# GiannisPikoulis/dsml-thesis

Hardware: AMD Instinct MI355X
Metric: DDIM denoise steps/sec (64×64×4 latent, 256² face) at 1/2/4/8 GPUs (higher is better)
Workload: dtype f32; 1 GPU; face_reenactment emotion-conditioned LDM (AffectNet config), DDIM-200 schedule, 16 samples/GPU, 64x64x4 latent, CFG off, eta 0, random-init weights; batch_per_gpu=16, global_batch=16, ddim_steps=200, hipgraph=True

## Files before the change

### dsml_thesis_amd/csrc/igemm.hip

```cpp
#include "ldmk_common.h"
#include <stdlib.h>
#include <type_traits>

#if defined(LDMK_IG_STAMPS) && (LDMK_IG_STAMPS == 1 || LDMK_IG_STAMPS == 3)
#define IG_T(i) do { const unsigned long long t_ = __builtin_amdgcn_s_memtime(); ig_acc[i] += t_ - ig_last; ig_last = t_; } while (0)
#elif defined(LDMK_IG_STAMPS)
#define IG_T(i) do { (void)ig_acc; (void)ig_last; } while (0)
#else
#define IG_T(i) do { } while (0)
#endif

namespace ldmk {

typedef __bf16 bf16x4 __attribute__((ext_vector_type(4)));
typedef __bf16 bf16x8 __attribute__((ext_vector_type(8)));
__device__ __forceinline__ bf16x4 to_bf16x4(const float4& v) {
  return bf16x4{(__bf16)v.x, (__bf16)v.y, (__bf16)v.z, (__bf16)v.w};
}

typedef _Float16 f16x4 __attribute__((ext_vector_type(4)));
typedef _Float16 f16x8 __attribute__((ext_vector_type(8)));
constexpr float H2_A_SCALE = 64.f;
__device__ __forceinline__ void split2h(const float4& v, f16x4& h, f16x4& l) {
  h = f16x4{(_Float16)v.x, (_Float16)v.y, (_Float16)v.z, (_Float16)v.w};
// ... 1298 lines not shown
               "ldmk_igemm: the fused skip connection needs a 3x3 convolution on a slab-GEMM tile, skip channels in multiples of 8");
  LDMK_REQUIRE(a.N % 4 == 0 && a.ldb % 4 == 0, "ldmk_igemm: N and ldb must be multiples of 4");
  LDMK_REQUIRE(a.rows_per_sample > 0, "ldmk_igemm: rows_per_sample");
  LDMK_REQUIRE((long long)a.M * a.ldc < (1LL << 31) && a.ldc > 0, "ldmk_igemm: output exceeds 2^31 elements per batch item (32-bit epilogue offsets)");
  const long long samples = ((long long)a.M + a.rows_per_sample - 1) / a.rows_per_sample;
  if (a.a_mode == LDMK_A_CONV3X3) {
    LDMK_REQUIRE(a.in_h > 0 && a.in_w > 0 && a.out_h > 0 && a.out_w > 0 && a.stride >= 1, "ldmk_igemm: conv geometry");
    LDMK_REQUIRE(a.rows_per_sample == a.out_h * a.out_w, "ldmk_igemm: rows_per_sample != out_h*out_w");
    LDMK_REQUIRE(a.batch <= 1, "ldmk_igemm: batched conv unsupported");
    LDMK_REQUIRE(samples * a.in_h * a.in_w * (a.c0 > a.c1 ? a.c0 : a.c1) < (1LL << 31),
                 "ldmk_igemm: conv input exceeds 2^31 elements (32-bit gather indices)");
  } else {
    LDMK_REQUIRE((long long)a.M * (a.c0 > a.c1 ? a.c0 : a.c1) < (1LL << 31), "ldmk_igemm: A exceeds 2^31 elements per batch item");
  }
  if (a.a_tf == LDMK_TF_AFFINE || a.a_tf == LDMK_TF_AFFINE_SILU) LDMK_REQUIRE(a.tf_coef, "ldmk_igemm: tf_coef missing");
  if (a.a_tf == LDMK_TF_LAYERNORM) {
    LDMK_REQUIRE(a.row_stats && a.ln_gamma && a.ln_beta && a.a_mode == LDMK_A_ROWS, "ldmk_igemm: layernorm prologue args");
  }
  if (a.a_tf == LDMK_TF_LAYERNORM_FOLDED)
    LDMK_REQUIRE(a.row_stats && a.ln_colsum && a.a_mode == LDMK_A_ROWS && !a.stats_out && a.batch <= 1,
                 "ldmk_igemm: folded layernorm needs row_stats, ln_colsum (ldmk_fold_layernorm), rows mode, no stats_out, no batching");
  LDMK_REQUIRE(a.a_tf >= LDMK_TF_NONE && a.a_tf <= LDMK_TF_LAYERNORM_FOLDED, "ldmk_igemm: a_tf=%d", a.a_tf);
  if (a.epi == LDMK_EPI_GEGLU) LDMK_REQUIRE(a.N % 64 == 0 && !a.residual && !a.batch_vec, "ldmk_igemm: GEGLU needs N%%64==0 and no residual");
  if (a.stats_out)
    LDMK_REQUIRE(a.M % 32 == 0 && a.rows_per_sample % 32 == 0 && a.epi == LDMK_EPI_NONE && a.batch <= 1,
                 "ldmk_igemm: stats_out needs M%%32==0, rows_per_sample%%32==0, no GEGLU, no batching");
  LDMK_REQUIRE(a.tile_cfg >= 0 && a.tile_cfg <= kNumCfg + kNumRCfg + kNumSCfg + kNumWCfg + kNumPCfg, "ldmk_igemm: tile_cfg=%d outside [0,%d]",
               a.tile_cfg, kNumCfg + kNumRCfg + kNumSCfg + kNumWCfg + kNumPCfg);
  LDMK_REQUIRE(a.splitk >= 0 && a.splitk <= 64, "ldmk_igemm: splitk=%d outside [0,64]", a.splitk);
  LDMK_REQUIRE(a.compute == LDMK_COMPUTE_F32 || a.compute == LDMK_COMPUTE_BF16 || a.compute == LDMK_COMPUTE_BF16X3 || a.compute == LDMK_COMPUTE_F16X2,
               "ldmk_igemm: compute=%d", a.compute);
  const bool ps_tile = a.tile_cfg > kNumCfg + kNumRCfg + kNumSCfg + kNumWCfg;
  if (a.compute == LDMK_COMPUTE_BF16X3 && !ps_tile) {
    LDMK_REQUIRE(a.w_split && !a.b_trans && a.w_split_ld >= a.K && a.w_split_ld % 8 == 0,
                 "ldmk_igemm: LDMK_COMPUTE_BF16X3 needs w_split (ldmk_pack_wsplit), b_trans = 0, w_split_ld >= K and a multiple of 8");
    LDMK_REQUIRE(3LL * a.N * a.w_split_ld * 2 < (1LL << 32), "ldmk_igemm: w_split exceeds 4 GB per batch entry");
    LDMK_REQUIRE(igemm_fast_gather_ok(a), "ldmk_igemm: LDMK_COMPUTE_BF16X3 needs the fast gather (no zero-insertion, two-source "
                 "upsampling or operands beyond 4 GB)");
  }
  if (a.compute == LDMK_COMPUTE_F16X2) {
    LDMK_REQUIRE(a.tile_cfg <= kNumCfg || ps_tile, "ldmk_igemm: LDMK_COMPUTE_F16X2 runs on the LDS-tiled shapes (tile_cfg 0..6) and the pre-split "
                 "tiles (23..28, 31..33), not tile_cfg=%d", a.tile_cfg);
    LDMK_REQUIRE(!a.a_split && a.w_scale_exp >= -60 && a.w_scale_exp <= 60, "ldmk_igemm: LDMK_COMPUTE_F16X2: a_split is not taken; w_scale_exp=%d", a.w_scale_exp);
    if (!ps_tile) {
      LDMK_REQUIRE(a.w_split && !a.b_trans && a.w_split_ld >= a.K && a.w_split_ld % 8 == 0 && 2LL * a.N * a.w_split_ld * 2 < (1LL << 32),
                   "ldmk_igemm: LDMK_COMPUTE_F16X2 needs w_split (ldmk_pack_wsplit_h2), b_trans = 0, w_split_ld >= K and a multiple of 8, below 4 GB");
// ... 97 lines not shown
```

### dsml_thesis_amd/csrc/igemm_ps.hip

```cpp
#include "ldmk_common.h"
#include <stdlib.h>

namespace ldmk {

typedef __bf16 pbf16x4 __attribute__((ext_vector_type(4)));
typedef __bf16 pbf16x8 __attribute__((ext_vector_type(8)));
typedef unsigned int pu32x4 __attribute__((ext_vector_type(4)));

#ifdef LDMK_PS_PROBES
constexpr bool PS_PROBES = true;
#else
constexpr bool PS_PROBES = false;
#endif
static int ps_probe_bits() {
  if (!PS_PROBES) return 0;
  const int dbg = ps_probe_bits();
  return dbg;
}

constexpr unsigned PS_OOB = 0x80000000u;

__device__ __forceinline__ pu32x4 ps_rsrc(const void* ptr, unsigned bytes) {
  const unsigned long long a = (unsigned long long)ptr;
  pu32x4 r;
// ... 1114 lines not shown
  *reinterpret_cast<pf16x8*>(d) = pf16x8{a0[0], a0[1], a0[2], a0[3], a1[0], a1[1], a1[2], a1[3]};
  *reinterpret_cast<pf16x8*>(d + 1024) = pf16x8{l0[0], l0[1], l0[2], l0[3], l1[0], l1[1], l1[2], l1[3]};
}

template <int NWM, int NWN, int TM, int TN, bool TR>
static int psc_launch(const ldmk_igemm_args& a, int splitk, float* ws, hipStream_t st) {
  constexpr int BM = 32 * TM * NWM, BN = 32 * TN * NWN;
  constexpr size_t lds = (size_t)3 * (BM / 32 + BN / 32) * 2048;
  static_assert(lds <= 160 * 1024, "LDS ring exceeds 160 KiB");
  static bool attr = false;
  if (!attr) {
    (void)hipFuncSetAttribute(reinterpret_cast<const void*>(igemm_psc_kernel<NWM, NWN, TM, TN, TR>), hipFuncAttributeMaxDynamicSharedMemorySize, (int)lds);
    attr = true;
  }
  const int tiles = ((a.M + BM - 1) / BM) * ((a.N + BN - 1) / BN);
  static const int nfast_env = [] { const char* e = getenv("LDMK_PS_NFAST"); return e ? atoi(e) : 1; }();
  static const int lean_env = [] { const char* e = getenv("LDMK_PS_LEAN"); return e ? atoi(e) : 1; }();
  const int nfast = (nfast_env && (a.N + BN - 1) / BN > 1 && (a.M + BM - 1) / BM >= 8 ? 1 : 0) | (lean_env ? 0 : 2);
  hipLaunchKernelGGL((igemm_psc_kernel<NWM, NWN, TM, TN, TR>), dim3(tiles, splitk, 1), dim3(64 * NWM * NWN), lds, st, a, splitk, ws, nfast);
  if (splitk > 1 && !a.raw_slabs) return launch_splitk_reduce(a, splitk, ws, st);
  return check_launch("ldmk_igemm(ps, conv)");
}

const char* igemm_ps_unsupported(const ldmk_igemm_args& a, int pcfg, int splitk) {
  if (a.compute != LDMK_COMPUTE_BF16X3 && a.compute != LDMK_COMPUTE_F16X2) return "the pre-split tiles run the bf16x3 and the f16x2 arithmetic (compute)";
  const int pl = a.compute == LDMK_COMPUTE_F16X2 ? 2 : 3;
  if (pl == 2 && (pcfg == 6 || pcfg == 7)) return "the warp-specialised pre-split tiles (29 / 30) exist in the bf16x3 arithmetic only";
  if (pl == 2 && a.out_ps && !a.range_flag) return "out_ps in the f16x2 arithmetic needs range_flag";
  if (!a.a_ps || !a.w_ps) return "a_ps / w_ps (operands in the PS layout: ldmk_pack_ps, ldmk_ln_stats_ps, out_ps of a producer GEMM)";
  if (a.a_mode == LDMK_A_CONV3X3) {
    if (pl != 2) return "the conv-mode pre-split tile runs the f16x2 arithmetic only";
    if (pcfg != 0 && pcfg != 1 && pcfg != 3 && pcfg != 4) return "conv mode: tile_cfg 23 / 24 / 26 / 27";
    if (a.c1 || a.a1 || a.upsample || a.a_tf != LDMK_TF_NONE || a.out_ps || a.batch > 1 || a.epi != LDMK_EPI_NONE || a.attn_kv_out)
      return "conv mode: one pre-normalised source (ldmk_gn_apply_ps_h2), no upsampling / prologue / out_ps / batching / GEGLU";
    if (a.c0 % 32) return "conv mode: C_in must be a multiple of 32";
    if ((a.c0 / 32) % splitk) return "conv mode: splitk must divide C_in / 32 (K is split on 32-channel chunk boundaries)";
    const long long smp = ((long long)a.M + a.rows_per_sample - 1) / a.rows_per_sample;
    if (((smp * a.in_h * a.in_w + 31) / 32) * (a.c0 / 16) * 2048 >= (1LL << 31)) return "conv mode: input of 2 GiB or more";
  } else if (a.a_mode != LDMK_A_ROWS) {
    return "rows mode or 3x3 convolution";
  }
  if (a.b_trans || a.upsample || a.skip_a0 || (a.splitk_counters && !(ps_probe_bits() & 8))) return "b_trans / upsample / fused skip / in-launch combine";
  if (a.a_tf != LDMK_TF_NONE && a.a_tf != LDMK_TF_LAYERNORM_FOLDED) return "no staging prologue: a_ps is what gets multiplied";
  if (a.K % 32 || a.N % 32) return "K and N must be multiples of 32";
  const long long kb = a.K / 16;
  if ((a.a_mode == LDMK_A_ROWS && (long long)((a.M + 31) / 32) * kb * pl * 1024 >= (1LL << 31)) || (long long)(a.N / 32) * kb * pl * 1024 >= (1LL << 31))
    return "an operand of 2 GiB or more";
  if (a.epi == LDMK_EPI_GEGLU && (!kPsCfg[pcfg].even_tn || splitk > 1)) return "GEGLU needs a tile of (value, gate) pairs (256x256, 128x256) and no split-K";
  if (splitk > a.K / 32) return "more K slices than 32-deep chunks";
  if (a.out_ps) {
    if (splitk > 1 || a.batch > 1 || a.stats_out) return "out_ps: no split-K, no batching, no GroupNorm records (transposed epilogue)";
    if (a.ldc % 16) return "out_ps: ldc (the PS output's column count) must be a multiple of 16";
  } else if (!a.out && splitk <= 1) {
    return "no output";
  }
  if (a.stats_out && !a.out) return "stats_out needs out";
  if (a.attn_kv_out) {
    if (pl != 2 || (pcfg != 0 && pcfg != 4)) return "attn_kv_out: the F16X2 arithmetic on tile_cfg 23 / 27";
    if (a.stats_out || splitk > 1 || a.batch > 1 || a.epi != LDMK_EPI_NONE || a.out_ps || !a.out || !a.range_flag)
      return "attn_kv_out: the fused QKV projection (no split-K / batching / GEGLU / records / out_ps; out and range_flag required)";
    if (a.attn_heads <= 0 || a.N != 3 * 32 * a.attn_heads) return "attn_kv_out: N must be 3 x 32 x attn_heads ([q | k | v] of d_head 32)";
    if (a.attn_tokens <= 0 || a.attn_tokens % 64 || a.M % a.attn_tokens) return "attn_kv_out: attn_tokens a multiple of 64 that divides M";
  }
  return nullptr;
}

int igemm_ps_dispatch(const ldmk_igemm_args& a, int pcfg, int splitk, float* ws, hipStream_t st) {
  const bool tr = !a.stats_out;
  if (a.a_mode == LDMK_A_CONV3X3) {
    switch (pcfg) {
      case 0: return tr ? psc_launch<8, 1, 1, 5, true>(a, splitk, ws, st) : psc_launch<8, 1, 1, 5, false>(a, splitk, ws, st);
      case 1: return tr ? psc_launch<4, 2, 2, 5, true>(a, splitk, ws, st) : psc_launch<4, 2, 2, 5, false>(a, splitk, ws, st);
      case 3: return tr ? psc_launch<4, 2, 1, 5, true>(a, splitk, ws, st) : psc_launch<4, 2, 1, 5, false>(a, splitk, ws, st);
      default: return tr ? psc_launch<4, 1, 1, 5, true>(a, splitk, ws, st) : psc_launch<4, 1, 1, 5, false>(a, splitk, ws, st);
    }
  }
  if (a.compute == LDMK_COMPUTE_F16X2 && a.attn_kv_out)
    return pcfg == 0 ? ps_launch<8, 1, 1, 5, 3, true, 2, true>(a, splitk, ws, st) : ps_launch<4, 1, 1, 5, 3, true, 2, true>(a, splitk, ws, st);
  if (a.compute == LDMK_COMPUTE_F16X2) {
    switch (pcfg) {
      case 0: return tr ? ps_launch<8, 1, 1, 5, 3, true, 2>(a, splitk, ws, st) : ps_launch<8, 1, 1, 5, 3, false, 2>(a, splitk, ws, st);
      case 1: return tr ? ps_launch<4, 2, 2, 5, 3, true, 2>(a, splitk, ws, st) : ps_launch<4, 2, 2, 5, 3, false, 2>(a, splitk, ws, st);
      case 2: return tr ? ps_launch<4, 2, 2, 4, 3, true, 2>(a, splitk, ws, st) : ps_launch<4, 2, 2, 4, 3, false, 2>(a, splitk, ws, st);
      case 3: return tr ? ps_launch<4, 2, 1, 5, 3, true, 2>(a, splitk, ws, st) : ps_launch<4, 2, 1, 5, 3, false, 2>(a, splitk, ws, st);
      case 4: return tr ? ps_launch<4, 1, 1, 5, 3, true, 2>(a, splitk, ws, st) : ps_launch<4, 1, 1, 5, 3, false, 2>(a, splitk, ws, st);
      case 8: return tr ? ps_launch<4, 1, 2, 5, 3, true, 2>(a, splitk, ws, st) : ps_launch<4, 1, 2, 5, 3, false, 2>(a, splitk, ws, st);
      case 9: return tr ? ps_launch<4, 1, 2, 4, 3, true, 2>(a, splitk, ws, st) : ps_launch<4, 1, 2, 4, 3, false, 2>(a, splitk, ws, st);
      case 10: return tr ? ps_launch<2, 2, 2, 4, 3, true, 2>(a, splitk, ws, st) : ps_launch<2, 2, 2, 4, 3, false, 2>(a, splitk, ws, st);
      default: return tr ? ps_launch<4, 2, 1, 4, 3, true, 2>(a, splitk, ws, st) : ps_launch<4, 2, 1, 4, 3, false, 2>(a, splitk, ws, st);
    }
// ... 106 lines not shown
```

### dsml_thesis_amd/engine.py

```python
import ctypes as C
import math
import os

import torch

from . import lib as L
from . import switches


def plan_key(a, m):
    key = f"{m},{a.N},{a.K},{a.a_mode},{a.a_tf},{a.epi},{max(1, a.batch)}"
    if a.b_trans:
        key += ",bt"
    if a.a_mode == L.A_CONV3X3 and (a.stride != 1 or a.upsample):
        key += f",s{a.stride}u{a.upsample}"
    return key


_SECTIONS = {"f32": "LDMK_PLAN_TABLE", "bf16x3": "LDMK_X3_TABLE", "f16x2": "LDMK_H2_TABLE", "ps_bf16x3": "LDMK_PS_TABLE",
             "ps_f16x2": "LDMK_PS_H2_TABLE"}
_TABLES = {}
_PLAN_FILE = os.path.join(os.path.dirname(os.path.abspath(__file__)), "igemm_plans.json")


# ... 570 lines not shown
        a._algo_flops = 2.0 * (4 * pix) * cout * (9 * c)
        if plan is not None:
            pg.igemm_ps(a, *plan)
        else:
            pg.igemm(a, self.pin, batch_is_samples=False)
        part = None
        out2d = out.view(-1, cout)
        if stats:
            self.drop_stats(out2d)
            part = self.stats_buffer(4 * pix, cout)
        pg.add("ldmk_upconv_scatter", p_(Pm), p_(bias), p_(out), p_(part), n, h, w, cout)
        if stats:
            self.attach_stats(out2d, part)
        pg.release(A, Pm)
        return out

    def _maybe_stats(self, a, out2d, rows_per_sample, stats):
        if stats and a.M % 32 == 0 and rows_per_sample % 32 == 0:
            self.drop_stats(out2d)
            part = self.stats_buffer(a.M, a.N)
            a.stats_out = part.data_ptr()
            self.attach_stats(out2d, part)

    def ps_query(self, M, N, K, tf=L.TF_NONE, epi=L.EPI_NONE, batch=1, per_sample=True):
        if not ps_enabled():
            return None
        m = M
        if self.pin is not None and self.pin[0] != self.pin[1] and per_sample:
            m = max(1, M * self.pin[0] // self.pin[1])
        return ps_plan(f"{N},{K},{L.A_ROWS},{tf},{epi},{max(1, batch)}", m, h2=getattr(self.pg, "h2_flag", None) is not None,
                       far=bool(getattr(self.pg, "far_plans", False)))

    def lin_ps(self, plan, M, K, a_ps, wp, w_ps, bias, rows_per_sample, out=None, out_ps=None, geglu=False, stats=False, **kw):
        pg, ops = self.pg, self.ops
        N = wp.shape[1]
        ncol = N // 2 if geglu else N
        if out is None and out_ps is None:
            out = pg.alloc(M, ncol)
        a = ops.make_igemm_args(M, N, K, None, K, wp, out, ncol, rows_per_sample, bias=bias,
                                epi=L.EPI_GEGLU if geglu else L.EPI_NONE, a_ps=a_ps, w_ps=w_ps, out_ps=out_ps,
                                range_flag=getattr(pg, "h2_flag", None), **kw)
        if out is not None:
            self._maybe_stats(a, out, rows_per_sample, stats)
        pg.igemm_ps(a, *plan)
        return out

    def lin(self, x0, wp, bias, rows_per_sample, x1=None, out=None, geglu=False, stats=False, wf=None, **kw):
        pg, ops = self.pg, self.ops
        M, c0 = x0.shape[0], x0.shape[-1]
        c1 = 0 if x1 is None else x1.shape[-1]
        N = wp.shape[1]
        ncol = N // 2 if geglu else N
# ... 29 lines not shown
```

### dsml_thesis_amd/lib.py

```python
import ctypes as C
import os

from . import switches

_HERE = os.path.dirname(os.path.abspath(__file__))
LIB_PATH = switches.get("LDMK_LIBRARY") or os.path.join(_HERE, "libldmk.so")

A_ROWS, A_CONV3X3 = 0, 1
TF_NONE, TF_AFFINE, TF_AFFINE_SILU, TF_LAYERNORM, TF_LAYERNORM_FOLDED = 0, 1, 2, 3, 4
EPI_NONE, EPI_GEGLU = 0, 1
COMPUTE_F32, COMPUTE_BF16, COMPUTE_BF16X3, COMPUTE_F16X2 = 0, 1, 2, 3
POST_NONE, POST_GROUPNORM, POST_LAYERNORM = 0, 1, 2

_fp = C.c_void_p


class IgemmArgs(C.Structure):
    _fields_ = [
        ("M", C.c_int), ("N", C.c_int), ("K", C.c_int),
        ("a0", _fp), ("a1", _fp), ("c0", C.c_int), ("c1", C.c_int),
        ("a_mode", C.c_int), ("in_h", C.c_int), ("in_w", C.c_int), ("out_h", C.c_int), ("out_w", C.c_int),
        ("stride", C.c_int), ("pad_lo", C.c_int), ("upsample", C.c_int),
        ("a_tf", C.c_int), ("tf_coef", _fp), ("row_stats", _fp), ("ln_gamma", _fp), ("ln_beta", _fp),
        ("rows_per_sample", C.c_int),
        ("w", _fp), ("b_trans", C.c_int), ("ldb", C.c_int),
        ("bias", _fp), ("batch_vec", _fp), ("batch_vec_ld", C.c_int),
        ("residual", _fp), ("epi", C.c_int),
        ("out", _fp), ("ldc", C.c_int), ("batch", C.c_int),
        ("a_bstride", C.c_longlong), ("w_bstride", C.c_longlong), ("out_bstride", C.c_longlong),
        ("alpha", C.c_float), ("tile_cfg", C.c_int), ("splitk", C.c_int),
        ("splitk_ws", _fp), ("splitk_ws_elems", C.c_longlong), ("stats_out", _fp), ("compute", C.c_int), ("splitk_counters", _fp), ("splitk_counters_len", C.c_int),
        ("w_frag", _fp),
        ("ln_colsum", _fp),
        ("raw_slabs", C.c_int),
        ("skip_a0", _fp), ("skip_a1", _fp), ("skip_c0", C.c_int), ("skip_c1", C.c_int),
        ("w_split", _fp), ("w_split_ld", C.c_int), ("w_split_bstride", C.c_longlong),
        ("a_split", _fp), ("a_split_ld", C.c_int),
        ("a_ps", _fp), ("a_ps_bstride", C.c_longlong), ("w_ps", _fp), ("w_ps_bstride", C.c_longlong), ("out_ps", _fp),
        ("w_scale_exp", C.c_int), ("range_flag", _fp),
        ("attn_kv_out", _fp), ("attn_tokens", C.c_int), ("attn_heads", C.c_int),
    ]


class PostArgs(C.Structure):
    _fields_ = [
        ("src", _fp), ("nslab", C.c_int), ("slab_stride", C.c_longlong), ("M", C.c_int), ("N", C.c_int),
        ("rows_per_sample", C.c_int), ("alpha", C.c_float), ("bias", _fp), ("batch_vec", _fp), ("batch_vec_ld", C.c_int),
        ("residual", _fp), ("ldr", C.c_int), ("geglu", C.c_int), ("raw_out", _fp), ("ld_raw", C.c_int), ("norm", C.c_int),
        ("x1", _fp), ("c1", C.c_int), ("groups", C.c_int), ("eps", C.c_float), ("gamma", _fp), ("beta", _fp),
        ("silu", C.c_int), ("norm_out", _fp), ("ld_norm", C.c_int), ("gn_cache_floats", C.c_int),
        ("gn_scratch", _fp), ("gn_scratch_elems", C.c_longlong),
    ]


class WgradArgs(C.Structure):
    _fields_ = [
        ("R", C.c_int), ("Kw", C.c_int), ("N", C.c_int), ("a", _fp), ("c", C.c_int), ("lda", C.c_int),
        ("a_mode", C.c_int), ("in_h", C.c_int), ("in_w", C.c_int), ("out_h", C.c_int), ("out_w", C.c_int),
        ("stride", C.c_int), ("pad_lo", C.c_int), ("upsample", C.c_int),
        ("dy", _fp), ("ldy", C.c_int), ("dw", _fp), ("ldw", C.c_int), ("accumulate", C.c_int), ("alpha", C.c_float),
        ("batch", C.c_int), ("a_bstride", C.c_longlong), ("dy_bstride", C.c_longlong), ("dw_bstride", C.c_longlong),
        ("splitr", C.c_int), ("ws", _fp), ("ws_elems", C.c_longlong), ("dbias", _fp), ("compute", C.c_int),
    ]
# ... 164 lines not shown
```

### dsml_thesis_amd/ops.py

```python
import ctypes as C
import math

import weakref

import torch

from . import lib as L


def _ptr(t):
    return 0 if t is None else (t if isinstance(t, int) else t.data_ptr())


def stream():
    return torch.cuda.current_stream().cuda_stream


def _chk(t, name):
    if t is None:
        return
    if not (t.is_cuda and t.dtype == torch.float32 and t.is_contiguous()):
        raise L.LdmkError(f"{name}: expected a contiguous float32 CUDA tensor, got {t.dtype} {t.device} "
                          f"contiguous={t.is_contiguous()}")

# ... 198 lines not shown
    a.geglu = 1 if geglu else 0
    a.raw_out, a.ld_raw = _ptr(raw_out), ((N // 2 if geglu else N) if ld_raw is None else ld_raw)
    a.norm, a.x1, a.c1, a.groups, a.eps = norm, _ptr(x1), c1, groups, float(eps)
    a.gamma, a.beta, a.silu = _ptr(gamma), _ptr(beta), 1 if silu else 0
    a.norm_out, a.ld_norm = _ptr(norm_out), ((N + c1) if ld_norm is None else ld_norm)
    return a


def post(args, device=None):
    need = L.load().ldmk_post_scratch_elems(C.byref(args))
    if need > 0 and not args.gn_scratch:
        scratch = torch.empty(need, device=device if device is not None else torch.device("cuda", torch.cuda.current_device()),
                              dtype=torch.float32)
        args.gn_scratch, args.gn_scratch_elems = scratch.data_ptr(), need
        args._scratch = scratch
    L.call("ldmk_post", C.byref(args), stream())


def make_igemm_args(M, N, K, a0, c0, w, out, ldc, rows_per_sample, a1=None, c1=0, conv=None, tf=L.TF_NONE,
                    tf_coef=None, row_stats=None, ln_gamma=None, ln_beta=None, b_trans=False, ldb=None, bias=None,
                    batch_vec=None, batch_vec_ld=0, residual=None, epi=L.EPI_NONE, batch=1, a_bstride=0, w_bstride=0,
                    out_bstride=0, alpha=1.0, splitk=0, splitk_ws=None, w_frag=None, tile_cfg=0, compute=0, ln_colsum=None,
                    splitk_counters=None, raw_slabs=False, a_split=None, w_bf16t=None, a_ps=None, w_ps=None, out_ps=None,
                    range_flag=None, attn_kv=None):
    a = L.IgemmArgs()
    a._keep = (a0, a1, w, out, tf_coef, row_stats, ln_gamma, ln_beta, bias, batch_vec, residual, splitk_ws, w_frag, ln_colsum,
               splitk_counters, a_split, w_bf16t, a_ps, w_ps, out_ps)
    a.M, a.N, a.K = M, N, K
    a.a0, a.a1, a.c0, a.c1 = _ptr(a0), _ptr(a1), c0, c1
    if conv is not None:
        a.a_mode = L.A_CONV3X3
        a.in_h, a.in_w, a.out_h, a.out_w, a.stride, a.pad_lo, a.upsample = conv
    else:
        a.a_mode = L.A_ROWS
    a.a_tf = tf
    a.tf_coef, a.row_stats, a.ln_gamma, a.ln_beta = _ptr(tf_coef), _ptr(row_stats), _ptr(ln_gamma), _ptr(ln_beta)
    a.rows_per_sample = rows_per_sample
    a.w, a.b_trans = _ptr(w), 1 if b_trans else 0
    a.ldb = ldb if ldb is not None else (K if b_trans else N)
    a.bias, a.batch_vec, a.batch_vec_ld = _ptr(bias), _ptr(batch_vec), batch_vec_ld
    a.residual, a.epi = _ptr(residual), epi
    a.out, a.ldc, a.batch = _ptr(out), ldc, batch
    a.a_bstride, a.w_bstride, a.out_bstride = a_bstride, w_bstride, out_bstride
    a.alpha = alpha
    a.splitk = splitk
    a.w_frag, a.tile_cfg, a.compute = _ptr(w_frag), tile_cfg, compute
    a.ln_colsum = _ptr(ln_colsum)
    a.raw_slabs = 1 if raw_slabs else 0
    if splitk_counters is not None:
        a.splitk_counters, a.splitk_counters_len = splitk_counters.data_ptr(), splitk_counters.numel()
    if splitk_ws is not None:
        a.splitk_ws, a.splitk_ws_elems = splitk_ws.data_ptr(), splitk_ws.numel()
    if w_bf16t is not None:
        a.w_split, a.w_split_ld = _ptr(w_bf16t), w_bf16t.shape[-1]
    if a_split is not None:
        a.a_split, a.a_split_ld = _ptr(a_split), a_split.shape[-1]
    if a_ps is not None:
        a.a_ps, a.w_ps, a.out_ps = _ptr(a_ps), _ptr(w_ps), _ptr(out_ps)
        if batch > 1:
            a.a_ps_bstride, a.w_ps_bstride = a_ps.shape[-1], w_ps.shape[-1]
        hit = _WPS_H2_EXP.get(w_ps.data_ptr())
        if hit is not None and hit[0]() is w_ps:
            a.compute, a.w_scale_exp, a.range_flag = L.COMPUTE_F16X2, hit[1], _ptr(range_flag)
            a._keep = a._keep + (range_flag,)
            if attn_kv is not None:
                a.attn_kv_out, a.attn_tokens, a.attn_heads = _ptr(attn_kv[0]), int(attn_kv[1]), int(attn_kv[2])
                a._keep = a._keep + (attn_kv[0],)
        else:
            a.compute = L.COMPUTE_BF16X3
        return a
    if compute == L.COMPUTE_BF16X3 and not set_split(a):
        raise ValueError("COMPUTE_BF16X3: no split images registered for this weight (ops.pack_wsplit) or b_trans set")
    if compute == L.COMPUTE_F16X2 and not set_split_h2(a, range_flag):
        raise ValueError("COMPUTE_F16X2: no fp16 images registered for this weight (ops.pack_wsplit_h2), b_trans set, or no range_flag")
    return a


def igemm(args):
    L.call("ldmk_igemm", C.byref(args), stream())


_SPLIT = {}


def pack_wsplit(w, batch=1):
    if batch > 1:
        assert w.dim() == 3 and w.shape[0] == batch and w.is_contiguous()
        K, N = w.shape[1], w.shape[2]
    else:
        assert w.dim() == 2 and w.is_contiguous()
# ... 340 lines not shown
```

### dsml_thesis_amd/switches.py

```python
import os

SWITCHES = {
    "LDMK_SPLIT_BF16": ("1", "arithmetic", "0: every GEMM and the attention on the f32 matrix-core form (v_mfma_f32_32x32x2_f32); the "
                        "f32_mfma_form leg of bench.py"),
    "LDMK_F16X2": ("1", "arithmetic", "0: split products from the exact bf16x3 split (six bf16 MFMAs, operands bit-exact) instead of "
                   "F16X2 (three fp16 MFMAs, range-checked per site); the bf16x3_form leg of bench.py"),
    "LDMK_LN_UNFOLDED": (None, "arithmetic", "set: LayerNorm applied in the GEMM prologue instead of folded through the product (what "
                         "the folded-LayerNorm guard switches a model to by itself)"),
    "LDMK_LN_GUARD_RATIO": ("4.0", "arithmetic", "|mean| / std of a token row above which the folded LayerNorm raises its guard"),
    "LDMK_ATTN_H2_MIN_TOKENS": ("512", "arithmetic", "self attention runs in F16X2 from this many tokens per sample, bf16x3 below"),
    "LDMK_H2_CONV_RULE": ("1", "arithmetic", "0: untabled long-K convolutions (K >= 1440) do not take the F16X2 rule"),
    "LDMK_PS": ("1", "route", "0: no pre-split (PS layout, LDS-DMA) GEMM tiles; same bits"),
    "LDMK_PSC": ("1", "route", "0: no conv-mode pre-split tile for 3x3 convolutions; same bits"),
    "LDMK_PSC_FORCE": (None, "route", "'cfg,splitk': force the conv-mode pre-split tile for every eligible convolution (A/B runs)"),
    "LDMK_POUT_PS": ("0", "route", "1: SpatialTransformer.proj_out on a pre-split tile instead of the row GEMM (measured slower)"),
    "LDMK_ATTN_PS": ("1", "route", "0: attn1.to_out does not read the attention result in the PS layout"),
    "LDMK_ATTN_PRESPLIT": ("1", "route", "0: K / V are split inside the attention kernel instead of once by their producer; same bits"),
    "LDMK_ATTN_PRESPLIT_MIN_TOKENS": ("2048", "route", "tokens per sample from which K / V are pre-split"),
    "LDMK_QKV_TILES": ("1", "route", "0: the fused QKV projection does not write the attention's K / V tiles from its epilogue"),
    "LDMK_NO_WINOGRAD": (None, "route", "set: no Winograd F(2x2,3x3) convolutions and no phase-split upsampling convolutions (direct "
                         "implicit GEMM everywhere; other bits, same tolerance)"),
    "LDMK_WINO_MIN_TILES": ("256", "route", "Winograd from this many 2x2 output tiles at the plan-policy batch"),
    "LDMK_WINO_MIN_CIN": ("320", "route", "Winograd / phase-split upsampling from this many input channels"),
    "LDMK_NO_SMALL_ROUTE": (None, "route", "set: batch 1-2 jobs run the batched launch program instead of the small-batch route"),
    "LDMK_SMALL_ROWS": ("4096", "route", "rows (batch x pixels at the policy batch) up to which the small-batch route is taken"),
    "LDMK_SPLITK_IN_LAUNCH": (None, "route", "set: split-K slabs combined by each tile's last workgroup instead of a reduce launch "
                              "(measured slower)"),
    "LDMK_TRAIN_NO_PACKED_W": (None, "route", "set: the training step's bf16 GEMMs read fp32 weights instead of the packed bf16 copies"),
    "LDMK_ATTN_QT": (None, "route", "1 | 2: query tiles per wave of the staged f32 attention kernel (A/B hook)"),
    "LDMK_NO_PLAN_TABLE": (None, "plan", "set: ignore igemm_plans.json (the library's built-in tile heuristic plans every GEMM)"),
    "LDMK_PLAN_MAX_RATIO": ("0", "plan", "> 0: a tuned plan is used only within this ratio of its tuned row count (0: nearest at any "
                            "distance)"),
    "LDMK_PLAN_TABLE": (None, "plan", "a file that replaces the `f32` section of igemm_plans.json (a flat {key: [cfg, splitk]} file as "
                        "the tuning tools write it, or another merged file whose section is taken)"),
    "LDMK_X3_TABLE": (None, "plan", "the same for the `bf16x3` section"),
    "LDMK_H2_TABLE": (None, "plan", "the same for the `f16x2` section"),
    "LDMK_PS_TABLE": (None, "plan", "the same for the `ps_bf16x3` section (pre-split tiles)"),
# ... 41 lines not shown
```

### dsml_thesis_amd/unet.py

```python
import math
import os

import torch
import torch.nn as nn

from . import lib as L
from . import switches
from . import ops
from .engine import ArithSites, NetBuilder, Program, far_from_tuned, split_enabled as engine_split_enabled, ps_enabled as engine_ps_enabled, f16x2_enabled

LN_GUARD_RATIO = float(switches.get("LDMK_LN_GUARD_RATIO", "4.0"))


ATTN_PRESPLIT_MIN_TOKENS = int(switches.get("LDMK_ATTN_PRESPLIT_MIN_TOKENS", "2048"))
ATTN_H2_MIN_TOKENS = int(switches.get("LDMK_ATTN_H2_MIN_TOKENS", "512"))


def ln_unfolded_default():
    return bool(switches.get("LDMK_LN_UNFOLDED"))


class _Params(nn.Module):
    def __init__(self, **shapes):
        super().__init__()
# ... 310 lines not shown
                     ln_beta=sd[q + "norm2.bias"], out=att, wf=P.get(q + "q2#f"))
        else:
            pg.add("ldmk_ln_stats_guard", p_(h1), rows, C_, 1e-5, p_(stats), LN_GUARD_RATIO, p_(ln_flag))
            q2 = lin(h1, P[q + "q2_ln"], P[q + "q2_ln#b"], hw, tf=L.TF_LAYERNORM_FOLDED, row_stats=stats,
                     ln_colsum=P[q + "q2_ln#cs"], out=att, wf=P.get(q + "q2_ln#f"))
        a2 = pg.alloc(rows, C_)
        if m.d_head == 32:
            pg.add("ldmk_attn_cross", p_(q2), C_, p_(kk), p_(vv), C_, p_(a2), C_, n, hw, L_ctx, m.heads, m.d_head ** -0.5)
        elif m.d_head in (40, 64, 80):
            pg.add("ldmk_attn_cross_d", p_(q2), C_, p_(kk), p_(vv), C_, p_(a2), C_, n, hw, L_ctx, m.heads, m.d_head, m.d_head ** -0.5)
        else:
            raise NotImplementedError(f"cross attention over a context of {L_ctx} tokens with heads of width {m.d_head} (built: 32, 40, 64, 80)")
        h2 = lin(a2, P[q + "o2"], sd[q + "attn2.to_out.0.bias"], hw, residual=h1, out=h1, wf=P.get(q + "o2#f"))
        nb_.release(att, a2)
        return h2

    def ff_section(q, h2, last):
        Nf = P[q + "ff2"].shape[0]
        plan_g = plan_f = None
        if not unfolded and q + "ff1_ln" + psfx() in P and q + "ff2" + psfx() in P:
            plan_g = nb_.ps_query(rows, 2 * Nf, C_, tf=L.TF_LAYERNORM_FOLDED, epi=L.EPI_GEGLU)
            plan_f = nb_.ps_query(rows, C_, Nf)
        if plan_g is not None and plan_f is not None:
            f_ps = pg.alloc_ps(rows, Nf)
            ln_lin(h2, q + "ff1_ln", True, out_ps=f_ps)
            plan_p = (nb_.ps_query(rows, m.ch, C_) if (last and prefix + "pout" + psfx() in P and plan_f[1] <= 1
                                                       and switches.get("LDMK_POUT_PS", "0") == "1") else None)
            hc_ps = pg.alloc_ps(rows, C_) if plan_p is not None else None
            hcur = nb_.lin_ps(plan_f, rows, Nf, f_ps, P[q + "ff2"], P[q + "ff2" + psfx()], sd[q + "ff.net.2.bias"], hw, out=h2, residual=h2,
                              out_ps=hc_ps)
            nb_.release(f_ps)
            return hcur, hc_ps, plan_p
        if unfolded:
            pg.add("ldmk_ln_stats", p_(h2), rows, C_, 1e-5, p_(stats))
            f = lin(h2, P[q + "ff1"], P[q + "ff1b"], hw, geglu=True, tf=L.TF_LAYERNORM, row_stats=stats,
                    ln_gamma=sd[q + "norm3.weight"], ln_beta=sd[q + "norm3.bias"], wf=P.get(q + "ff1#f"))
        else:
            f = ln_lin(h2, q + "ff1_ln", True)
        hcur = lin(f, P[q + "ff2"], sd[q + "ff.net.2.bias"], hw, residual=h2, out=h2, wf=P.get(q + "ff2#f"))
        nb_.release(f)
        return hcur, None, None

    for d in range(m.depth):
        q = f"{prefix}transformer_blocks.{d}."
        with nb_.site(q + "attn1"):
            h1, att = attn1_section(q, hcur)
        if L_ctx == 1:
            h2 = h1
        else:
            with nb_.site(q + "attn2"):
                h2 = attn2_section(q, h1, att)
        ff_site = q + "ff"
        with nb_.site(ff_site):
            hcur, hc_ps, plan_p = ff_section(q, h2, d == m.depth - 1)
    if hc_ps is not None:
        with nb_.site(ff_site):
            out = nb_.lin_ps(plan_p, rows, C_, hc_ps, P[prefix + "pout"], P[prefix + "pout" + psfx()], sd[prefix + "proj_out.bias"], hw, residual=xr,
                             stats=True)
        nb_.release(hc_ps)
    else:
        with nb_.site(prefix + "proj_out"):
            out = lin(hcur, P[prefix + "pout"], sd[prefix + "proj_out.bias"], hw, residual=xr, stats=True, wf=P.get(prefix + "pout#f"))
    nb_.release(hcur, stats)
    return out.view(n, h, w, m.ch)


MAX_ARITHMETIC_PASSES = 5


def rerun_if_flags_tripped(unet_of):
    import functools

    def deco(fn):
        @functools.wraps(fn)
        def wrapped(self, *args, **kwargs):
            if torch.cuda.is_current_stream_capturing():
                return fn(self, *args, **kwargs)
            unet = unet_of(self)
            rng = torch.cuda.get_rng_state()
            for _ in range(MAX_ARITHMETIC_PASSES):
                out = fn(self, *args, **kwargs)
                if not unet.flags_tripped():
                    break
                torch.cuda.set_rng_state(rng)
            return out
        return wrapped
    return deco

# ... 513 lines not shown
```

### include/ldmk.h

```cpp
#ifndef LDMK_H
#define LDMK_H
#ifdef __cplusplus
extern "C" {
#endif

#define LDMK_OK 0
#define LDMK_EINVAL (-1)
#define LDMK_EHIP (-2)
#define LDMK_ENOMEM (-3)

int ldmk_version(void);
const char* ldmk_last_error(void);
int ldmk_init(int device);

enum { LDMK_A_ROWS = 0, LDMK_A_CONV3X3 = 1 };
enum { LDMK_TF_NONE = 0, LDMK_TF_AFFINE = 1, LDMK_TF_AFFINE_SILU = 2, LDMK_TF_LAYERNORM = 3,
       LDMK_TF_LAYERNORM_FOLDED = 4 };
enum { LDMK_EPI_NONE = 0, LDMK_EPI_GEGLU = 1 };
enum { LDMK_COMPUTE_F32 = 0, LDMK_COMPUTE_BF16 = 1, LDMK_COMPUTE_BF16X3 = 2, LDMK_COMPUTE_F16X2 = 3 };
#define LDMK_F16X2_A_EXP 6
#define LDMK_F16X2_RANGE 1000.0f

typedef struct ldmk_igemm_args {
  int M, N, K;
  const float* a0;
  const float* a1;
  int c0, c1;
  int a_mode;
  int in_h, in_w;
  int out_h, out_w;
  int stride, pad_lo;
  int upsample;
  int a_tf;
  const float* tf_coef;
  const float* row_stats;
  const float* ln_gamma;
  const float* ln_beta;
  int rows_per_sample;
  const float* w;
  int b_trans, ldb;
  const float* bias;
// ... 15 lines not shown
  int* splitk_counters;
  int splitk_counters_len;
  const float* w_frag;
  const float* ln_colsum;
  int raw_slabs;
  const float* skip_a0;
  const float* skip_a1;
  int skip_c0, skip_c1;
  const void* w_split;
  int w_split_ld;
  long long w_split_bstride;
  const void* a_split;
  int a_split_ld;
  const void* a_ps;
  long long a_ps_bstride;
  const void* w_ps;
  long long w_ps_bstride;
  void* out_ps;
  int w_scale_exp;
  int* range_flag;
  void* attn_kv_out;
  int attn_tokens;
  int attn_heads;
} ldmk_igemm_args;

long long ldmk_ps_bytes(int rows, int k);
int ldmk_pack_ps(const float* src, int rows, int k, long long row_stride, long long k_stride, int batch, long long src_bstride,
                 void* dst, void* stream);
int ldmk_ln_stats_ps(const float* x, int rows, int c, float eps, float* stats, void* dst, float guard, int* flag, void* stream);

long long ldmk_ps_bytes_h2(int rows, int k);
int ldmk_pack_ps_h2(const float* src, int rows, int k, long long row_stride, long long k_stride, int batch, long long src_bstride,
                    int scale_exp, int* range_flag, void* dst, void* stream);
int ldmk_ln_stats_ps_h2(const float* x, int rows, int c, float eps, float* stats, void* dst, float guard, int* flag, int* range_flag,
                        void* stream);
int ldmk_gn_apply_ps_h2(const float* x0, int c0, const float* x1, int c1, const float* coef, void* y_ps, int n, int hw, int silu,
                        int* range_flag, void* stream);

int ldmk_pack_wsplit(const float* w, int K, int N, int ldb, int batch, long long w_bstride, void* out, int ld_out, void* stream);
int ldmk_pack_wsplit_h2(const float* w, int K, int N, int ldb, int batch, long long w_bstride, int scale_exp, void* out, int ld_out,
                        void* stream);
int ldmk_pack_wbf16t(const float* w, int K, int N, int ldb, void* out, int ld_out, void* stream);

int ldmk_igemm(const ldmk_igemm_args* args, void* stream);
long long ldmk_igemm_workspace_elems(const ldmk_igemm_args* args);
int ldmk_igemm_check(const ldmk_igemm_args* args);
// ... 201 lines not shown
```

Baseline: 1135 sample-steps/s.

## Fuse transformer feed-forward GEGLU and ff.net.2 into one pre-split kernel

Adds a fused f16x2 kernel for the SpatialTransformer feed-forward when C=160. It computes the LN-folded GEGLU projection per 64-column chunk, applies GELU gating in registers, splits the result to f16 hi/lo and feeds it straight into the second GEMM accumulators. This removes the round trip of the hidden activation through global memory and one launch. The cost is the weight streaming through a double-buffered LDS ring with one wave per 32 rows, which may give lower occupancy and parallelism than the separate tiled GEMMs. It only applies to transformer blocks with 32768 or more rows.

After: 1141 sample-steps/s, median of 6. No clear change (+0.5%).

```diff
diff --git a/dsml_thesis_amd/csrc/igemm.hip b/dsml_thesis_amd/csrc/igemm.hip
--- a/dsml_thesis_amd/csrc/igemm.hip
+++ b/dsml_thesis_amd/csrc/igemm.hip
@@ -1344,6 +1344,9 @@
                  "ldmk_igemm: folded layernorm needs row_stats, ln_colsum (ldmk_fold_layernorm), rows mode, no stats_out, no batching");
   LDMK_REQUIRE(a.a_tf >= LDMK_TF_NONE && a.a_tf <= LDMK_TF_LAYERNORM_FOLDED, "ldmk_igemm: a_tf=%d", a.a_tf);
   if (a.epi == LDMK_EPI_GEGLU) LDMK_REQUIRE(a.N % 64 == 0 && !a.residual && !a.batch_vec, "ldmk_igemm: GEGLU needs N%%64==0 and no residual");
+  LDMK_REQUIRE(a.epi >= LDMK_EPI_NONE && a.epi <= LDMK_EPI_GEGLU_FF, "ldmk_igemm: epi=%d", a.epi);
+  LDMK_REQUIRE(a.epi != LDMK_EPI_GEGLU_FF || a.tile_cfg > kNumCfg + kNumRCfg + kNumSCfg + kNumWCfg,
+               "ldmk_igemm: the fused feed-forward (LDMK_EPI_GEGLU_FF) runs on a pre-split tile_cfg (23..33)");
   if (a.stats_out)
     LDMK_REQUIRE(a.M % 32 == 0 && a.rows_per_sample % 32 == 0 && a.epi == LDMK_EPI_NONE && a.batch <= 1,
                  "ldmk_igemm: stats_out needs M%%32==0, rows_per_sample%%32==0, no GEGLU, no batching");
diff --git a/dsml_thesis_amd/csrc/igemm_ps.hip b/dsml_thesis_amd/csrc/igemm_ps.hip
--- a/dsml_thesis_amd/csrc/igemm_ps.hip
+++ b/dsml_thesis_amd/csrc/igemm_ps.hip
@@ -1160,7 +1160,217 @@
   return check_launch("ldmk_igemm(ps, conv)");
 }
 
+template <int C>
+__global__ __launch_bounds__(256, 1) void ffn_h2_kernel(const ldmk_igemm_args p) {
+  constexpr int NW = 4;
+  constexpr int KS1 = C / 16, CB = C / 32;
+  constexpr int U1 = 2 * KS1, U = U1 + 2 * CB;
+  constexpr int UHI = (U + NW - 1) / NW;
+  constexpr int STAGE = U * 2048;
+  extern __shared__ __attribute__((aligned(1024))) unsigned char smem_ps[];
+
+  const int tid = threadIdx.x, lane = tid & 63, wave = __builtin_amdgcn_readfirstlane(tid >> 6);
+  const int l31 = lane & 31, half = lane >> 5;
+  const int Mb = (p.M + 31) / 32;
+  const int blk = blockIdx.x * NW + wave;
+  const int row = blk * 32 + l31;
+  const bool rok = row < p.M;
+  const int Nf = p.ff_hidden, nch = Nf / 32, Kb2 = Nf / 16;
+  const unsigned lane16 = lane * 16;
+  const unsigned lds0 = (unsigned)(size_t)smem_ps;
+
+  const pu32x4 rs1 = ps_rsrc(p.w_ps, (unsigned)Kb2 * (unsigned)KS1 * 2048u);
+  const pu32x4 rs2 = ps_rsrc(p.w2_ps, (unsigned)CB * (unsigned)Kb2 * 2048u);
+  auto issue = [&](int j) {
+    const unsigned buf = lds0 + (unsigned)(j & 1) * STAGE;
+#pragma unroll
+    for (int i = 0; i < UHI; ++i) {
+      const int u = wave + NW * i;
+      if (u < U) {
+        unsigned off;
+        if (u < U1) {
+          off = j < nch ? (unsigned)(2 * j * KS1 + u) * 2048u : PS_OOB;
+        } else {
+          const int v = u - U1;
+          off = j >= 1 ? (unsigned)((v >> 1) * Kb2 + 2 * (j - 1) + (v & 1)) * 2048u : PS_OOB;
+        }
+        ps_dma<2>(lane16 + off, u < U1 ? rs1 : rs2, buf + (unsigned)u * 2048u);
+      }
+    }
+  };
+  issue(0);
+
+  float* vcs = reinterpret_cast<float*>(smem_ps + 2 * STAGE);
+  float* vb1 = vcs + 2 * Nf;
+  for (int i = tid; i < Nf / 2; i += 64 * NW) {
+    reinterpret_cast<float4*>(vcs)[i] = reinterpret_cast<const float4*>(p.ln_colsum)[i];
+    reinterpret_cast<float4*>(vb1)[i] = reinterpret_cast<const float4*>(p.bias)[i];
+  }
+  const int rr = rok ? row : p.M - 1;
+  const float2 st = reinterpret_cast<const float2*>(p.row_stats)[rr];
+  const float mean = st.x, rstd = st.y;
+  const float alpha1 = p.alpha;
+  const float alpha2 = ldexpf(1.f, -(LDMK_F16X2_A_EXP + p.w2_scale_exp));
+
+  pf16x8 ah[KS1], al[KS1];
+  {
+    const unsigned char* ap = reinterpret_cast<const unsigned char*>(p.a_ps) + (size_t)min(blk, Mb - 1) * KS1 * 2048 + lane16;
+#pragma unroll
+    for (int s = 0; s < KS1; ++s) {
+      ah[s] = *reinterpret_cast<const pf16x8*>(ap + s * 2048);
+      al[s] = *reinterpret_cast<const pf16x8*>(ap + s * 2048 + 1024);
+    }
+  }
+  __syncthreads();
+
+  f32x16 acc2[CB];
+#pragma unroll
+  for (int n = 0; n < CB; ++n)
+#pragma unroll
+    for (int r = 0; r < 16; ++r) acc2[n][r] = 0.f;
+  bool bad = false;
+
+  auto gemm1 = [&](const unsigned char* sb, f32x16& av, f32x16& ag) {
+#pragma unroll
+    for (int r = 0; r < 16; ++r) { av[r] = 0.f; ag[r] = 0.f; }
+#pragma unroll
+    for (int s = 0; s < KS1; ++s) {
+      const pf16x8 vh = *reinterpret_cast<const pf16x8*>(sb + s * 2048), vl = *reinterpret_cast<const pf16x8*>(sb + s * 2048 + 1024);
+      const pf16x8 gh = *reinterpret_cast<const pf16x8*>(sb + (KS1 + s) * 2048), gl = *reinterpret_cast<const pf16x8*>(sb + (KS1 + s) * 2048 + 1024);
+      av = __builtin_amdgcn_mfma_f32_32x32x16_f16(vh, al[s], av, 0, 0, 0);
+      av = __builtin_amdgcn_mfma_f32_32x32x16_f16(vl, ah[s], av, 0, 0, 0);
+      av = __builtin_amdgcn_mfma_f32_32x32x16_f16(vh, ah[s], av, 0, 0, 0);
+      ag = __builtin_amdgcn_mfma_f32_32x32x16_f16(gh, al[s], ag, 0, 0, 0);
+      ag = __builtin_amdgcn_mfma_f32_32x32x16_f16(gl, ah[s], ag, 0, 0, 0);
+      ag = __builtin_amdgcn_mfma_f32_32x32x16_f16(gh, ah[s], ag, 0, 0, 0);
+    }
+  };
+  auto geglu = [&](const f32x16& av, const f32x16& ag, const int jc, pf16x8 (&hh)[2], pf16x8 (&hl)[2]) {
+    typedef unsigned pu32x2 __attribute__((ext_vector_type(2)));
+    pu32x2 xh[4], xl[4];
+#pragma unroll
+    for (int q = 0; q < 4; ++q) {
+      const int c = 64 * jc + 8 * q + 4 * half;
+      const float4 cs = *reinterpret_cast<const float4*>(vcs + c), bi = *reinterpret_cast<const float4*>(vb1 + c);
+      const float4 csg = *reinterpret_cast<const float4*>(vcs + c + 32), big = *reinterpret_cast<const float4*>(vb1 + c + 32);
+      float4 v = make_float4(av[4 * q] * alpha1, av[4 * q + 1] * alpha1, av[4 * q + 2] * alpha1, av[4 * q + 3] * alpha1);
+      float4 g = make_float4(ag[4 * q] * alpha1, ag[4 * q + 1] * alpha1, ag[4 * q + 2] * alpha1, ag[4 * q + 3] * alpha1);
+      v.x = ps_lnf_bias(v.x, mean, cs.x, rstd, bi.x); v.y = ps_lnf_bias(v.y, mean, cs.y, rstd, bi.y);
+      v.z = ps_lnf_bias(v.z, mean, cs.z, rstd, bi.z); v.w = ps_lnf_bias(v.w, mean, cs.w, rstd, bi.w);
+      g.x = ps_lnf_bias(g.x, mean, csg.x, rstd, big.x); g.y = ps_lnf_bias(g.y, mean, csg.y, rstd, big.y);
+      g.z = ps_lnf_bias(g.z, mean, csg.z, rstd, big.z); g.w = ps_lnf_bias(g.w, mean, csg.w, rstd, big.w);
+      v.x *= gelu_erf_f(g.x); v.y *= gelu_erf_f(g.y); v.z *= gelu_erf_f(g.z); v.w *= gelu_erf_f(g.w);
+      v.x += 0.f; v.y += 0.f; v.z += 0.f; v.w += 0.f;
+      bad |= rok && ps_h2_out_of_range(v);
+      pf16x4 h, l;
+      ps_split2h(ps_scaled_sat(v), h, l);
+      xh[q] = __builtin_bit_cast(pu32x2, h);
+      xl[q] = __builtin_bit_cast(pu32x2, l);
+    }
+#pragma unroll
+    for (int s = 0; s < 2; ++s) {
+      const auto h0 = __builtin_amdgcn_permlane32_swap(xh[2 * s].x, xh[2 * s + 1].x, false, false);
+      const auto h1 = __builtin_amdgcn_permlane32_swap(xh[2 * s].y, xh[2 * s + 1].y, false, false);
+      const auto l0 = __builtin_amdgcn_permlane32_swap(xl[2 * s].x, xl[2 * s + 1].x, false, false);
+      const auto l1 = __builtin_amdgcn_permlane32_swap(xl[2 * s].y, xl[2 * s + 1].y, false, false);
+      hh[s] = __builtin_bit_cast(pf16x8, pu32x4{h0[0], h1[0], h0[1], h1[1]});
+      hl[s] = __builtin_bit_cast(pf16x8, pu32x4{l0[0], l1[0], l0[1], l1[1]});
+    }
+  };
+  auto gemm2 = [&](const unsigned char* sb2, const pf16x8 (&hh)[2], const pf16x8 (&hl)[2]) {
+#pragma unroll
+    for (int s = 0; s < 2; ++s)
+#pragma unroll
+      for (int n = 0; n < CB; ++n) {
+        const pf16x8 wh = *reinterpret_cast<const pf16x8*>(sb2 + (2 * n + s) * 2048), wl = *reinterpret_cast<const pf16x8*>(sb2 + (2 * n + s) * 2048 + 1024);
+        acc2[n] = __builtin_amdgcn_mfma_f32_32x32x16_f16(wh, hl[s], acc2[n], 0, 0, 0);
+        acc2[n] = __builtin_amdgcn_mfma_f32_32x32x16_f16(wl, hh[s], acc2[n], 0, 0, 0);
+        acc2[n] = __builtin_amdgcn_mfma_f32_32x32x16_f16(wh, hh[s], acc2[n], 0, 0, 0);
+      }
+  };
+  auto stage = [&](int j) -> const unsigned char* {
+    ps_wait_vm<0>();
+    asm volatile("s_barrier" ::: "memory");
+    if (j < nch) issue(j + 1);
+    return smem_ps + (j & 1) * STAGE + lane16;
+  };
+
+  f32x16 pv, pg;
+  gemm1(stage(0), pv, pg);
+  for (int j = 1; j < nch; ++j) {
+    const unsigned char* sb = stage(j);
+    f32x16 av, ag;
+    pf16x8 hh[2], hl[2];
+    gemm1(sb, av, ag);
+    geglu(pv, pg, j - 1, hh, hl);
+    gemm2(sb + U1 * 2048, hh, hl);
+    pv = av;
+    pg = ag;
+#pragma unroll
+    for (int i = 0; i < 6 * KS1; ++i) {
+      __builtin_amdgcn_sched_group_barrier(0x008, 1, 0);
+      __builtin_amdgcn_sched_group_barrier(0x002, 5, 0);
+    }
+  }
+  {
+    const unsigned char* sb = stage(nch);
+    pf16x8 hh[2], hl[2];
+    geglu(pv, pg, nch - 1, hh, hl);
+    gemm2(sb + U1 * 2048, hh, hl);
+  }
+  ps_wait_vm<0>();
+
+  if (rok) {
+    float* __restrict__ outp = p.out + (long long)row * p.ldc;
+    const float* __restrict__ resp = p.residual + (long long)row * p.ldc;
+#pragma unroll
+    for (int n = 0; n < CB; ++n)
+#pragma unroll
+      for (int q = 0; q < 4; ++q) {
+        const int col = 32 * n + 8 * q + 4 * half;
+        const float4 b2 = *reinterpret_cast<const float4*>(p.bias2 + col), rs = *reinterpret_cast<const float4*>(resp + col);
+        float4 v = make_float4(acc2[n][4 * q] * alpha2, acc2[n][4 * q + 1] * alpha2, acc2[n][4 * q + 2] * alpha2, acc2[n][4 * q + 3] * alpha2);
+        v.x = ps_bias_res(v.x, b2.x, 0.f, rs.x); v.y = ps_bias_res(v.y, b2.y, 0.f, rs.y);
+        v.z = ps_bias_res(v.z, b2.z, 0.f, rs.z); v.w = ps_bias_res(v.w, b2.w, 0.f, rs.w);
+        *reinterpret_cast<float4*>(outp + col) = v;
+      }
+  }
+  if (bad) *p.range_flag = 1;
+}
+
+constexpr int kFfnC = 160;
+static size_t ffn_lds(int ff_hidden) { return (size_t)2 * (2 * (kFfnC / 16) + 2 * (kFfnC / 32)) * 2048 + (size_t)16 * ff_hidden; }
+
+static int ffn_launch(const ldmk_igemm_args& a, hipStream_t st) {
+  static bool attr = false;
+  if (!attr) {
+    (void)hipFuncSetAttribute(reinterpret_cast<const void*>(ffn_h2_kernel<kFfnC>), hipFuncAttributeMaxDynamicSharedMemorySize, 160 * 1024);
+    attr = true;
+  }
+  const int wgs = ((a.M + 31) / 32 + 3) / 4;
+  hipLaunchKernelGGL(ffn_h2_kernel<kFfnC>, dim3(wgs), dim3(256), ffn_lds(a.ff_hidden), st, a);
+  return check_launch("ldmk_igemm(ffn)");
+}
+
+static const char* ffn_unsupported(const ldmk_igemm_args& a, int splitk) {
+  if (a.compute != LDMK_COMPUTE_F16X2 || !a.range_flag) return "the fused feed-forward runs the f16x2 arithmetic (compute) and needs range_flag";
+  if (splitk > 1) return "the fused feed-forward does not split K";
+  if (a.a_mode != LDMK_A_ROWS || a.a_tf != LDMK_TF_LAYERNORM_FOLDED || !a.a_ps || !a.w_ps || !a.bias || !a.ln_colsum)
+    return "the fused feed-forward: rows mode, folded LayerNorm, a_ps / w_ps / bias / ln_colsum";
+  if (a.K != kFfnC) return "the fused feed-forward is built for K = 160";
+  if (!a.w2_ps || !a.bias2 || !a.out || !a.residual || a.ff_hidden <= 0 || a.ff_hidden % 32 || a.N != 2 * a.ff_hidden)
+    return "the fused feed-forward: w2_ps, bias2, out, residual; ff_hidden a multiple of 32, N = 2 ff_hidden";
+  if (a.w2_scale_exp < -60 || a.w2_scale_exp > 60) return "w2_scale_exp outside [-60, 60]";
+  if (ffn_lds(a.ff_hidden) > 160 * 1024) return "the fused feed-forward: ff_hidden too large for LDS";
+  if (a.ldc < a.K || a.ldc % 4 || a.batch > 1 || a.out_ps || a.stats_out || a.batch_vec || a.attn_kv_out || a.upsample || a.b_trans || a.c1 ||
+      a.skip_a0 || a.raw_slabs || a.splitk_counters)
+    return "the fused feed-forward: ldc >= K and a multiple of 4; no batching / out_ps / records / per-sample vector / K / V tiles";
+  if ((long long)((a.M + 31) / 32) * (a.K / 16) * 2048 >= (1LL << 31) || (long long)a.N * a.K * 4 >= (1LL << 31)) return "an operand of 2 GiB or more";
+  return nullptr;
+}
+
 const char* igemm_ps_unsupported(const ldmk_igemm_args& a, int pcfg, int splitk) {
+  if (a.epi == LDMK_EPI_GEGLU_FF) return ffn_unsupported(a, splitk);
   if (a.compute != LDMK_COMPUTE_BF16X3 && a.compute != LDMK_COMPUTE_F16X2) return "the pre-split tiles run the bf16x3 and the f16x2 arithmetic (compute)";
   const int pl = a.compute == LDMK_COMPUTE_F16X2 ? 2 : 3;
   if (pl == 2 && (pcfg == 6 || pcfg == 7)) return "the warp-specialised pre-split tiles (29 / 30) exist in the bf16x3 arithmetic only";
@@ -1204,6 +1414,7 @@
 }
 
 int igemm_ps_dispatch(const ldmk_igemm_args& a, int pcfg, int splitk, float* ws, hipStream_t st) {
+  if (a.epi == LDMK_EPI_GEGLU_FF) return ffn_launch(a, st);
   const bool tr = !a.stats_out;
   if (a.a_mode == LDMK_A_CONV3X3) {
     switch (pcfg) {
diff --git a/dsml_thesis_amd/engine.py b/dsml_thesis_amd/engine.py
--- a/dsml_thesis_amd/engine.py
+++ b/dsml_thesis_amd/engine.py
@@ -616,12 +616,15 @@
             a.stats_out = part.data_ptr()
             self.attach_stats(out2d, part)
 
+    def policy_rows(self, M):
+        if self.pin is not None and self.pin[0] != self.pin[1]:
+            return max(1, M * self.pin[0] // self.pin[1])
+        return M
+
     def ps_query(self, M, N, K, tf=L.TF_NONE, epi=L.EPI_NONE, batch=1, per_sample=True):
         if not ps_enabled():
             return None
-        m = M
-        if self.pin is not None and self.pin[0] != self.pin[1] and per_sample:
-            m = max(1, M * self.pin[0] // self.pin[1])
+        m = self.policy_rows(M) if per_sample else M
         return ps_plan(f"{N},{K},{L.A_ROWS},{tf},{epi},{max(1, batch)}", m, h2=getattr(self.pg, "h2_flag", None) is not None,
                        far=bool(getattr(self.pg, "far_plans", False)))
 
diff --git a/dsml_thesis_amd/lib.py b/dsml_thesis_amd/lib.py
--- a/dsml_thesis_amd/lib.py
+++ b/dsml_thesis_amd/lib.py
@@ -8,7 +8,7 @@
 
 A_ROWS, A_CONV3X3 = 0, 1
 TF_NONE, TF_AFFINE, TF_AFFINE_SILU, TF_LAYERNORM, TF_LAYERNORM_FOLDED = 0, 1, 2, 3, 4
-EPI_NONE, EPI_GEGLU = 0, 1
+EPI_NONE, EPI_GEGLU, EPI_GEGLU_FF = 0, 1, 2
 COMPUTE_F32, COMPUTE_BF16, COMPUTE_BF16X3, COMPUTE_F16X2 = 0, 1, 2, 3
 POST_NONE, POST_GROUPNORM, POST_LAYERNORM = 0, 1, 2
 
@@ -39,6 +39,7 @@
         ("a_ps", _fp), ("a_ps_bstride", C.c_longlong), ("w_ps", _fp), ("w_ps_bstride", C.c_longlong), ("out_ps", _fp),
         ("w_scale_exp", C.c_int), ("range_flag", _fp),
         ("attn_kv_out", _fp), ("attn_tokens", C.c_int), ("attn_heads", C.c_int),
+        ("w2_ps", _fp), ("bias2", _fp), ("ff_hidden", C.c_int), ("w2_scale_exp", C.c_int),
     ]
 
 
diff --git a/dsml_thesis_amd/ops.py b/dsml_thesis_amd/ops.py
--- a/dsml_thesis_amd/ops.py
+++ b/dsml_thesis_amd/ops.py
@@ -244,7 +244,7 @@
                     batch_vec=None, batch_vec_ld=0, residual=None, epi=L.EPI_NONE, batch=1, a_bstride=0, w_bstride=0,
                     out_bstride=0, alpha=1.0, splitk=0, splitk_ws=None, w_frag=None, tile_cfg=0, compute=0, ln_colsum=None,
                     splitk_counters=None, raw_slabs=False, a_split=None, w_bf16t=None, a_ps=None, w_ps=None, out_ps=None,
-                    range_flag=None, attn_kv=None):
+                    range_flag=None, attn_kv=None, w2_ps=None, bias2=None):
     a = L.IgemmArgs()
     a._keep = (a0, a1, w, out, tf_coef, row_stats, ln_gamma, ln_beta, bias, batch_vec, residual, splitk_ws, w_frag, ln_colsum,
                splitk_counters, a_split, w_bf16t, a_ps, w_ps, out_ps)
@@ -288,6 +288,12 @@
             if attn_kv is not None:
                 a.attn_kv_out, a.attn_tokens, a.attn_heads = _ptr(attn_kv[0]), int(attn_kv[1]), int(attn_kv[2])
                 a._keep = a._keep + (attn_kv[0],)
+            if w2_ps is not None:
+                hit2 = _WPS_H2_EXP.get(w2_ps.data_ptr())
+                if hit2 is None or hit2[0]() is not w2_ps:
+                    raise ValueError("EPI_GEGLU_FF: w2_ps must come from pack_wps(..., h2=True)")
+                a.w2_ps, a.bias2, a.ff_hidden, a.w2_scale_exp = _ptr(w2_ps), _ptr(bias2), N // 2, hit2[1]
+                a._keep = a._keep + (w2_ps, bias2)
         else:
             a.compute = L.COMPUTE_BF16X3
         return a
diff --git a/dsml_thesis_amd/switches.py b/dsml_thesis_amd/switches.py
--- a/dsml_thesis_amd/switches.py
+++ b/dsml_thesis_amd/switches.py
@@ -13,6 +13,7 @@
     "LDMK_PS": ("1", "route", "0: no pre-split (PS layout, LDS-DMA) GEMM tiles; same bits"),
     "LDMK_PSC": ("1", "route", "0: no conv-mode pre-split tile for 3x3 convolutions; same bits"),
     "LDMK_PSC_FORCE": (None, "route", "'cfg,splitk': force the conv-mode pre-split tile for every eligible convolution (A/B runs)"),
+    "LDMK_FFN_FUSED": ("1", "route", "0: the transformer feed-forward as two pre-split launches (GEGLU, ff.net.2) instead of one; same bits"),
     "LDMK_POUT_PS": ("0", "route", "1: SpatialTransformer.proj_out on a pre-split tile instead of the row GEMM (measured slower)"),
     "LDMK_ATTN_PS": ("1", "route", "0: attn1.to_out does not read the attention result in the PS layout"),
     "LDMK_ATTN_PRESPLIT": ("1", "route", "0: K / V are split inside the attention kernel instead of once by their producer; same bits"),
diff --git a/dsml_thesis_amd/unet.py b/dsml_thesis_amd/unet.py
--- a/dsml_thesis_amd/unet.py
+++ b/dsml_thesis_amd/unet.py
@@ -356,10 +356,21 @@
             plan_g = nb_.ps_query(rows, 2 * Nf, C_, tf=L.TF_LAYERNORM_FOLDED, epi=L.EPI_GEGLU)
             plan_f = nb_.ps_query(rows, C_, Nf)
         if plan_g is not None and plan_f is not None:
+            pout_ps = (last and prefix + "pout" + psfx() in P and plan_f[1] <= 1 and switches.get("LDMK_POUT_PS", "0") == "1")
+            if (hf() is not None and not pout_ps and plan_f[1] <= 1 and C_ == FFN_FUSED_C
+                    and nb_.policy_rows(rows) >= FFN_FUSED_MIN_ROWS and switches.get("LDMK_FFN_FUSED", "1") != "0"):
+                wkey = q + "ff1_ln"
+                xs = pg.alloc_ps(rows, C_)
+                pg.add("ldmk_ln_stats_ps_h2", p_(h2), rows, C_, 1e-5, p_(stats), p_(xs), LN_GUARD_RATIO, p_(ln_flag), p_(hf()))
+                a = ops.make_igemm_args(rows, 2 * Nf, C_, None, C_, P[wkey], h2, C_, hw, bias=P[wkey + "#b"], epi=L.EPI_GEGLU_FF,
+                                        tf=L.TF_LAYERNORM_FOLDED, row_stats=stats, ln_colsum=P[wkey + "#cs"], residual=h2, a_ps=xs,
+                                        w_ps=P[wkey + psfx()], range_flag=hf(), w2_ps=P[q + "ff2" + psfx()], bias2=sd[q + "ff.net.2.bias"])
+                pg.igemm_ps(a, *plan_g)
+                nb_.release(xs)
+                return h2, None, None
             f_ps = pg.alloc_ps(rows, Nf)
             ln_lin(h2, q + "ff1_ln", True, out_ps=f_ps)
-            plan_p = (nb_.ps_query(rows, m.ch, C_) if (last and prefix + "pout" + psfx() in P and plan_f[1] <= 1
-                                                       and switches.get("LDMK_POUT_PS", "0") == "1") else None)
+            plan_p = nb_.ps_query(rows, m.ch, C_) if pout_ps else None
             hc_ps = pg.alloc_ps(rows, C_) if plan_p is not None else None
             hcur = nb_.lin_ps(plan_f, rows, Nf, f_ps, P[q + "ff2"], P[q + "ff2" + psfx()], sd[q + "ff.net.2.bias"], hw, out=h2, residual=h2,
                               out_ps=hc_ps)
@@ -398,6 +409,9 @@
     nb_.release(hcur, stats)
     return out.view(n, h, w, m.ch)
 
+
+FFN_FUSED_C = 160
+FFN_FUSED_MIN_ROWS = 32768
 
 MAX_ARITHMETIC_PASSES = 5
 
diff --git a/include/ldmk.h b/include/ldmk.h
--- a/include/ldmk.h
+++ b/include/ldmk.h
@@ -16,7 +16,8 @@
 enum { LDMK_A_ROWS = 0, LDMK_A_CONV3X3 = 1 };
 enum { LDMK_TF_NONE = 0, LDMK_TF_AFFINE = 1, LDMK_TF_AFFINE_SILU = 2, LDMK_TF_LAYERNORM = 3,
        LDMK_TF_LAYERNORM_FOLDED = 4 };
-enum { LDMK_EPI_NONE = 0, LDMK_EPI_GEGLU = 1 };
+enum { LDMK_EPI_NONE = 0, LDMK_EPI_GEGLU = 1,
+       LDMK_EPI_GEGLU_FF = 2 };
 enum { LDMK_COMPUTE_F32 = 0, LDMK_COMPUTE_BF16 = 1, LDMK_COMPUTE_BF16X3 = 2, LDMK_COMPUTE_F16X2 = 3 };
 #define LDMK_F16X2_A_EXP 6
 #define LDMK_F16X2_RANGE 1000.0f
@@ -78,6 +79,10 @@
   void* attn_kv_out;
   int attn_tokens;
   int attn_heads;
+  const void* w2_ps;
+  const float* bias2;
+  int ff_hidden;
+  int w2_scale_exp;
 } ldmk_igemm_args;
 
 long long ldmk_ps_bytes(int rows, int k);
```
